# junfeng-chen/position_induced_transformer

Hardware: AMD Instinct MI355X
Metric: PiT fwd+bwd samples/sec on Darcy2D (higher is better)
Workload: dtype f32; 1 GPU; darcy2d 43x43 grid->16x16 latent, pit_fixed hid64 H2 blocks4 loc0.02, RelL2 (train_darcy.py:64-111), fwd+loss+bwd, per-GPU batch 8; per_gpu_batch=8, global_batch=8, parallelism=single, launch=hipgraph, head_scale_route=host

## Files before the change

### include/pit_hip.h

```cpp
#ifndef PIT_HIP_H
#define PIT_HIP_H

#ifdef __cplusplus
extern "C" {
#endif

#define PIT_ABI_VERSION 31
#define PIT_MAX_SPACE_DIM 8
#define PIT_DSCALE_SLOTS 1024

#define PIT_METRIC_EUCLID     0
#define PIT_METRIC_PERIODIC1D 1
#define PIT_METRIC_PERIODIC2D 2

#define PIT_ERR_NULL     -1
#define PIT_ERR_SIZE     -2
#define PIT_ERR_METRIC   -3
#define PIT_ERR_UNSUPPORTED -4

int pit_version(void);
const char* pit_error_string(int code);

#define PIT_MATH_FP32 0
#define PIT_MATH_BF16 1
// ... 339 lines not shown
                                   float* d_values, long ld_dvalues, long dvalues_bstride,
                                   const int* nbr_cnt, int nbr_cap, int coord_dims, void* stream);

int pit_distmat_select_fwd(const float* m, long ld_m, long m_bstride, int mesh_batch, int n_out, int n_in,
                           int rank_k, int need_kth, float* stats, void* stream);
int pit_distmat_fwd(const float* m, long ld_m, long m_bstride, int n_out, int n_in,
                    const float* values, int batch, int dim, long ld_values, long values_bstride,
                    const float* head, int n_head, int head_is_scale,
                    const float* stats, float rank_w, int masked,
                    float* out, long ld_out, long out_bstride, int out_col0, int copy_inputs,
                    float* rowstat, float* scale_out, int math_mode, void* stream);
long pit_distmat_bwd_workspace(int batch, int n_out, int n_head);
int pit_distmat_bwd(const float* m, long ld_m, long m_bstride, int n_out, int n_in,
                    const float* values, int batch, int dim, long ld_values, long values_bstride,
                    const float* head, int n_head, int head_is_scale, const float* scale,
                    const float* rowstat, int masked,
                    const float* d_out, long ld_dout, long dout_bstride, int out_col0,
                    float* d_values, long ld_dvalues, long dvalues_bstride, int add_residual,
                    float* d_head, int accumulate_head, double* workspace,
                    float* d_m, const float* out, long ld_out, long out_bstride, float* a_workspace,
                    int math_mode, void* stream);

#define PIT_HAS_DISTLIST 1
#define PIT_DISTLIST_MAX_CAP 2048
#define PIT_DISTLIST_CHUNK 512
#define PIT_DISTLIST_CHUNK_SLOTS(n_out, cap) ((long)(n_out) * (long)(cap) / (PIT_DISTLIST_CHUNK / 2) + 1)
int pit_distlist_select_fwd(const int* idx, const float* sqd, long ld, long bstride, int cap, int mesh_batch, int n_out, int n_in,
                            int rank_k, int need_kth, float* stats, void* stream);
int pit_distlist_fwd(const int* idx, const float* sqd, long ld, long bstride, int cap, int n_out, int n_in,
                     const float* values, int batch, int dim, long ld_values, long values_bstride,
                     const float* head, int n_head, int head_is_scale,
                     const float* stats, float rank_w, int masked,
                     float* out, long ld_out, long out_bstride, int out_col0, int copy_inputs,
                     float* rowstat, float* scale_out, int math_mode, void* stream);
long pit_distlist_bwd_workspace(int batch, int n_out, int cap, int dim);
int pit_distlist_bwd(const int* idx, const float* sqd, long ld, long bstride, int cap, int n_out, int n_in,
                     const float* values, int batch, int dim, long ld_values, long values_bstride,
                     const float* head, int n_head, int head_is_scale, const float* scale,
                     const float* rowstat, int masked,
                     const float* d_out, long ld_dout, long dout_bstride, int out_col0,
                     float* d_values, long ld_dvalues, long dvalues_bstride, int add_residual,
                     float* d_head, int accumulate_head, double* workspace,
                     float* d_sqd, const float* out, long ld_out, long out_bstride,
                     const int* rev_ptr, const int* rev_pos, const int* chunk_ptr, const int* chunk_key, float* dv_workspace,
                     int math_mode, void* stream);

#define PIT_HAS_RAGGED_STEP 1
int pit_rel_lp_loss_ragged_fwd_grad(const float* tru, const float* pred, const int* len, int batch, int npts, int nch, int p,
                                    float* norms, float* loss, unsigned* workspace, float* d_pred_unit, float* clear_buf,
                                    long clear_n, void* stream);
int pit_rel_max_norm_ragged(const float* tru, const float* pred, const int* len, int batch, int npts, int nch, float* out,
                            void* stream);

int pit_debug_mfma_tile(const float* a, const float* b, float* d, void* stream);

#define PIT_RIDER_OWN          0
#define PIT_RIDER_PAIR_DW      1
#define PIT_RIDER_PAIR_WIDE    2
#define PIT_RIDER_SPARSE_PAIR  3
#define PIT_RIDER_SPARSE_ROWS  4
#define PIT_RIDER_DHEAD_FINISH 5
#define PIT_RIDER_BLOCK        6
#define PIT_RIDER_BLOCK2       7
#define PIT_RIDER_SATT         8
#define PIT_RIDER_KINDS        9
int pit_debug_rider_counts(int* out, int n, int reset);

#define PIT_GEMM_RD_TN1            0
#define PIT_GEMM_RD_TN2            1
#define PIT_GEMM_RD_PAIR           2
#define PIT_GEMM_RD_TRIPLE_TN1     3
#define PIT_GEMM_RD_TRIPLE_TN2     4
#define PIT_GEMM_LDS_32            5
#define PIT_GEMM_LDS_64            6
#define PIT_GEMM_LDS_128           7
#define PIT_GEMM_LDS_AGZ           8
#define PIT_GEMM_BFL_32            9
#define PIT_GEMM_BFL_64           10
#define PIT_GEMM_BFL_128          11
#define PIT_GEMM_BFL_IO16         12
#define PIT_GEMM_RR               13
#define PIT_GEMM_RR_PAIR          14
#define PIT_GEMM_MUL_GELU_GRAD    15
#define PIT_GEMM_THIN_DZ1         16
#define PIT_GEMM_THIN_FWD         17
#define PIT_GEMM_THIN_FWD_STREAM  18
#define PIT_GEMM_THIN_DW          19
#define PIT_GEMM_MLP_FWD16        20
#define PIT_GEMM_MLP_BWD16        21
#define PIT_GEMM_MLP_FWD64        22
#define PIT_GEMM_MLP_FWD64_THIN   23
#define PIT_GEMM_MLP_BWD64        24
#define PIT_GEMM_MLP_BWD64_THIN   25
#define PIT_GEMM_LAST_FWD16       26
#define PIT_GEMM_LAST_BWD16       27
#define PIT_GEMM_LAST_FWD64       28
#define PIT_GEMM_LAST_BWD64       29
#define PIT_GEMM_KINDS            30
int pit_debug_gemm_counts(int* out, int n, int reset);

#ifdef __cplusplus
}
#endif
#endif
```

### position_induced_transformer_amd/_lib.py

```python
from __future__ import annotations

import ctypes
import os

import torch

_HERE = os.path.dirname(os.path.abspath(__file__))
LIB_PATH = os.environ.get("PIT_LIB_PATH") or os.path.join(_HERE, "csrc", "libpit_hip.so")

_P = ctypes.c_void_p
_I = ctypes.c_int
_L = ctypes.c_long
_F = ctypes.c_float

class MlpParamsJob(ctypes.Structure):
    _fields_ = [("x", _P), ("ldx", _L), ("rows", _I), ("n0", _I), ("n1", _I), ("n2", _I), ("h", _P), ("out_gelu", _I),
                ("d_y", _P), ("ld_dy", _L), ("d_w1", _P), ("d_b1", _P), ("d_w2", _P), ("d_b2", _P),
                ("accumulate", _I), ("scratch", _P), ("math_mode", _I)]


class BlockWeightsJob(ctypes.Structure):
    _fields_ = [("mesh", _P), ("n_pts", _I), ("space_dim", _I), ("metric", _I), ("period", _F),
                ("n_layers", _I), ("heads", _P), ("head_is_scale", _I), ("n_head", _I),
                ("e", _P), ("q", _P), ("inv", _P), ("rowstat", _P), ("scale_out", _P)]
# ... 102 lines not shown
    "pit_union_att_supported": [_I, _I, _I, _I],
    "pit_union_att_fwd": [_P, _P, _L, _L, _I, _I, _I, _P, _P, _L, _L, _I, _I, _P],
    "pit_union_att_bwd": [_P, _P, _L, _L, _I, _I, _I, _P, _P, _P, _L, _L, _I, _P, _L, _L, _P, _I, _P],
    "pit_encoder_fwd": [_P, _P, _I, _I, _P, _L, _L, _I, _I, _I, _I, _P, _I, _P, _P, _P, _P,
                        _P, _P, _P, _P, _P, _L, _P, _P, _P, _L, _P, _P, _P],
    "pit_encoder_bwd": [_P, _P, _I, _I, _P, _L, _L, _I, _I, _I, _I, _P, _P, _P, _P, _P, _P, _P, _L, _P, _P, _P],
    "pit_posatt_pre_supported": [_I, _I, _I, _I],
    "pit_posatt_pre_fwd": [_P, _P, _I, _I, _I, _I, _P, _L, _L, _P, _L, _L, _I, _I, _I, _P],
    "pit_posatt_pre_bwd": [_P, _P, _P, _I, _I, _I, _I, _P, _L, _L, _P, _L, _L, _I, _P, _L, _L, _I, _P, _I, _P],
    "pit_block_bwd": [_P, _P, _P, _I, _I, _I, _I, _P, _P, _P, _P, _P, _P, _P, _I, _I, _P, _L, _P, _P, _L, _P, _P, _I, _P],
    "pit_mlp_bf16_io_supported": [_I, _I, _I, _I, _I],
    "pit_mlp_fwd": [_P, _L, _I, _I, _I, _I, _P, _P, _P, _P, _I, _P, _P, _P, _P, _L, _I, _P],
    "pit_mlp_bwd": [_P, _L, _I, _I, _I, _I, _P, _P, _P, _P, _P, _I, _P, _L,
                    _P, _L, _P, _P, _P, _P, _I, _P, _I, _P],
    "pit_mlp_bwd_data": [_I, _I, _I, _I, _P, _P, _P, _P, _I, _P, _L, _P, _L, _P, _I, _P],
    "pit_mlp_bwd_params": [_P, _L, _I, _I, _I, _I, _P, _I, _P, _L, _P, _P, _P, _P, _I, _P, _I, _P],
    "pit_mlp_bwd_params_ordered": [_P, _L, _I, _I, _I, _I, _P, _I, _P, _L, _P, _P, _P, _P, _I, _P, _P, _P],
    "pit_mlp_bwd_params_ordered_workspace": [_I, _I, _I, _I],
    "pit_mlp_bwd_params_ordered_mfma": [_P, _L, _I, _I, _I, _I, _P, _I, _P, _L, _P, _P, _P, _P, _I, _P, _P, _P],
    "pit_mlp_bwd_params_ordered_mfma_workspace": [_I, _I, _I, _I],
    "pit_lists_sort_ranges": [_P, _P, _I, _I, _L, _P, _P],
    "pit_posatt_overflow_dv_ordered": [_P, _P, _I, _I, _I, _I, _I, _F, _I, _I, _P, _I, _I, _P, _P,
                                       _P, _L, _L, _I, _P, _L, _L, _P, _I, _I, _P],
    "pit_mlp_bwd_params_deferrable": [_I, _I, _I, _I, _I, _L],
    "pit_rel_lp_loss_fwd": [_P, _P, _P, _P, _I, _I, _I, _I, _P, _P, _P, _P],
    "pit_rel_lp_loss_fwd_grad": [_P, _P, _P, _P, _I, _I, _I, _I, _P, _P, _P, _P, _P, _P, _L, _P],
    "pit_rel_lp_loss_fwd_grad_ordered": [_P, _P, _P, _P, _I, _I, _I, _I, _P, _P, _P, _P, _P, _P, _L, _P],
    "pit_rel_lp_loss_bwd": [_P, _P, _P, _P, _I, _I, _I, _I, _P, _P, _P, _P, _P],
    "pit_plan_ragged_fwd": [_P, _P, _I, _I, _I, _I, _P, _P, _F, _I, _P, _P, _I, _P, _P, _P],
    "pit_posatt_ragged_fwd": _RAGGED + _FWD_RAGGED,
    "pit_posatt_ragged_bwd": _RAGGED + _BWD_RAGGED,
    "pit_plan_ragged_strided_fwd": [_P, _P, _I, _I, _I, _I, _L, _L, _P, _P, _F, _I, _P, _P, _I, _P, _P, _P],
    "pit_posatt_ragged_strided_fwd": _RAGGED_STRIDED + _FWD_RAGGED,
    "pit_posatt_ragged_strided_bwd": _RAGGED_STRIDED + _BWD_RAGGED,
    "pit_rel_lp_loss_ragged_fwd": [_P, _P, _P, _I, _I, _I, _I, _P, _P, _P],
    "pit_rel_lp_loss_ragged_bwd": [_P, _P, _P, _I, _I, _I, _I, _P, _P, _P, _P],
    "pit_rel_lp_loss_ragged_fwd_grad": [_P, _P, _P, _I, _I, _I, _I, _P, _P, _P, _P, _P, _L, _P],
    "pit_rel_max_norm_ragged": [_P, _P, _P, _I, _I, _I, _P, _P],
    "pit_distmat_select_fwd": [_P, _L, _L, _I, _I, _I, _I, _I, _P, _P],
    "pit_distmat_fwd": _MAT + _FWD_DIST,
    "pit_distmat_bwd_workspace": [_I, _I, _I],
    "pit_distmat_bwd": _MAT + _BWD_DIST + [_P] + _SAVED_OUT + [_P] + _TAIL,
    "pit_distlist_select_fwd": [_P, _P, _L, _L, _I, _I, _I, _I, _I, _I, _P, _P],
    "pit_distlist_fwd": _LIST + _FWD_DIST,
    "pit_distlist_bwd_workspace": [_I, _I, _I, _I],
    "pit_distlist_bwd": _LIST + _BWD_DIST + [_P] + _SAVED_OUT + [_P] * 5 + _TAIL,
    "pit_rel_max_norm": [_P, _P, _I, _I, _I, _P, _P, _P],
    "pit_instance_norm_fwd": [_P, _L, _L, _I, _I, _I, _F, _P, _P, _P],
    "pit_instance_norm_bwd": [_P, _P, _P, _I, _I, _I, _P, _P],
    "pit_adam_step": [_P, _P, _P, _P, _L, _P, _F, _F, _I, _F, _F, _F, _F, _I, _P, _P],
    "pit_debug_mfma_tile": [_P, _P, _P, _P],
    "pit_debug_rider_counts": [_P, _I, _I],
    "pit_debug_gemm_counts": [_P, _I, _I],
}

LONG_RETURN = {"pit_satt_tiles_elems", "pit_posatt_dmesh_workspace", "pit_mlp_bwd_params_ordered_workspace",
               "pit_mlp_bwd_params_ordered_mfma_workspace", "pit_distmat_bwd_workspace", "pit_distlist_bwd_workspace"}
ADDED_LATER = {"pit_distlist_select_fwd", "pit_distlist_fwd", "pit_distlist_bwd_workspace", "pit_distlist_bwd",
               "pit_rel_lp_loss_ragged_fwd_grad", "pit_rel_max_norm_ragged"}
DISTLIST_CHUNK = 512


def distlist_chunk_slots(n_out: int, cap: int) -> int:
    return int(n_out) * int(cap) // (DISTLIST_CHUNK // 2) + 1
ABI_VERSION = 31

_lib = None


def lib() -> ctypes.CDLL:
    global _lib
    if _lib is None:
        if not os.path.exists(LIB_PATH):
            raise RuntimeError(
                f"{LIB_PATH} not found: build it with `python -m position_induced_transformer_amd.build` "
                "(hipcc --offload-arch=gfx950). There is no CPU or PyTorch fallback for the PiT hot path.")
        handle = ctypes.CDLL(LIB_PATH)
        for name, argtypes in SIGNATURES.items():
            try:
                fn = getattr(handle, name)
            except AttributeError:
                if name not in ADDED_LATER:
                    raise
                raise RuntimeError(f"{LIB_PATH} was built before {name} joined PIT_ABI_VERSION {ABI_VERSION}: "
                                   "rebuild it (python -m position_induced_transformer_amd.build)") from None
            fn.argtypes = argtypes
            fn.restype = ctypes.c_char_p if name == "pit_error_string" else (_L if name in LONG_RETURN else _I)
        got = handle.pit_version()
        if got != ABI_VERSION:
            raise RuntimeError(f"{LIB_PATH} implements PIT_ABI_VERSION {got}, this package binds version {ABI_VERSION}: "
                               "rebuild it (python -m position_induced_transformer_amd.build)")
        _lib = handle
    return _lib


def check(code: int, what: str) -> None:
    if code != 0:
        msg = lib().pit_error_string(code)
        raise RuntimeError(f"{what} failed ({code}): {msg.decode() if msg else '?'}")


def stream_ptr() -> int:
    return torch.cuda.current_stream().cuda_stream


def ptr(t) -> int:
    return 0 if t is None else t.data_ptr()


def values_args(t, with_batch: bool) -> tuple:
    b, _, d = t.shape
    return (t.data_ptr(),) + ((b, d) if with_batch else (d,)) + (t.stride(1), t.stride(0))
# ... 25 lines not shown
```

### position_induced_transformer_amd/csrc/pit_block.hip

```cpp
#include "pit_common.h"
#include "pit_gemm_rd.h"
#include "pit_block_dev.h"
#include <cstdlib>

namespace {

#ifdef PIT_STAMPS
__device__ unsigned long long pit_block_stamps[32];
#define BSTAMP(i_) do { if (blockIdx.x == 5 && threadIdx.x == 0) pit_block_stamps[i_] = __builtin_amdgcn_s_memtime(); } while (0)
#else
#define BSTAMP(i_) do { } while (0)
#endif

#ifdef PIT_WGREC
__device__ unsigned long long pit_block_wgrec[1024 * 4];
#define BREC(slot_) do { if (threadIdx.x == 0 && blockIdx.x < 1024) {                                                       \
        pit_block_wgrec[blockIdx.x * 4 + (slot_)] = __builtin_amdgcn_s_memrealtime();                                       \
        if ((slot_) == 0) { pit_block_wgrec[blockIdx.x * 4 + 2] = __builtin_amdgcn_s_getreg((4 << 0) | (0 << 6) | (31 << 11));   \
                            pit_block_wgrec[blockIdx.x * 4 + 3] = __builtin_amdgcn_s_getreg((20 << 0) | (0 << 6) | (31 << 11)); } } } while (0)
#else
#define BREC(slot_) do { } while (0)
#endif
#ifdef PIT_STAMPS_DBG
__device__ int pit_block_dbg = 0;
#define PIT_BLOCK_DBG pit_block_dbg
#else
#define PIT_BLOCK_DBG 0
#endif
#ifndef PIT_BLOCK_EXP
#define PIT_BLOCK_EXP 0
#endif

__global__ __launch_bounds__(256) void block_weights_kernel(WeightsArgs a) { block_weights_body(a, blockIdx.x); }

template <int NH, bool SHARED>
__device__ __forceinline__ void slab_contract(const float* __restrict__ w, long wstride, int L, const float* __restrict__ v,
                                              long ldv, int vhead, const float* __restrict__ sc, int jb, int je, int l15, int kq,
                                              f32x4_t (&acc)[SHARED ? NH : 1][4]) {
    constexpr int NS = SHARED ? 2 : 1;
    const float* wp = w + (long)l15 * L + 4 * kq;
    const float* vp = v + 4 * l15;
    for (int j0 = jb; j0 < je; j0 += 16 * NS) {
        float4 av[NH][NS], sv[NH][NS], bv[SHARED ? 1 : NH][NS][4];
        const int dbg = PIT_BLOCK_DBG;
#pragma unroll
        for (int h = 0; h < NH; ++h)
#pragma unroll
            for (int s = 0; s < NS; ++s) {
                av[h][s] = (dbg & 4) ? make_float4(1.f, 2.f, 3.f, 4.f) : *reinterpret_cast<const float4*>(wp + h * wstride + j0 + 16 * s);
                if (!SHARED) sv[h][s] = *reinterpret_cast<const float4*>(sc + (long)h * L + j0 + 16 * s + 4 * kq);
            }
#pragma unroll
        for (int h = 0; h < (SHARED ? 1 : NH); ++h)
#pragma unroll
            for (int s = 0; s < NS; ++s)
#pragma unroll
                for (int m = 0; m < 4; ++m)
                    bv[h][s][m] = (dbg & 2) ? make_float4(1.f, 2.f, 3.f, 4.f)
                                            : *reinterpret_cast<const float4*>(vp + h * vhead + (long)(j0 + 16 * s + 4 * kq + m) * ldv);
        __builtin_amdgcn_sched_barrier(0);
#pragma unroll
        for (int s = 0; s < NS; ++s)
#pragma unroll
            for (int m = 0; m < 4; ++m)
#pragma unroll
                for (int h = 0; h < NH; ++h) {
                    if ((PIT_BLOCK_EXP & (SHARED ? 1 : 4)) && (SHARED ? s == 1 : h == 1)) {
                        asm volatile("" :: "v"(av[h][s].x), "v"(av[h][s].y), "v"(av[h][s].z), "v"(av[h][s].w));
                        asm volatile("" :: "v"(bv[SHARED ? 0 : h][s][m].x), "v"(bv[SHARED ? 0 : h][s][m].y), "v"(bv[SHARED ? 0 : h][s][m].z), "v"(bv[SHARED ? 0 : h][s][m].w));
                        if (!SHARED) asm volatile("" :: "v"(sv[h][s].x), "v"(sv[h][s].y), "v"(sv[h][s].z), "v"(sv[h][s].w));
                        continue;
                    }
                    const float* ap = &av[h][s].x;
                    const float* sp = &sv[h][s].x;
                    const float aw = SHARED ? ap[m] : ap[m] * sp[m];
                    const float4 bb = bv[SHARED ? 0 : h][s][m];
                    f32x4_t (&ac)[4] = acc[SHARED ? h : 0];
                    ac[0] = mfma_16x16x4(aw, bb.x, ac[0]);
                    ac[1] = mfma_16x16x4(aw, bb.y, ac[1]);
                    ac[2] = mfma_16x16x4(aw, bb.z, ac[2]);
                    ac[3] = mfma_16x16x4(aw, bb.w, ac[3]);
                }
    }
}

__device__ __forceinline__ bool slab_of(int id, int batch, int slabs, int& sample, int& slab) {
    if (PIT_BLOCK_DBG & 1) return slab_of_linear(id, batch, slabs, sample, slab);
    return slab_of_xcd(id, batch, slabs, sample, slab);
}

struct BlockFwdArgs {
    const float *e, *inv;
    int L, batch;
    float* xcat;
    const float *w1, *b1, *w2, *b2;
    int out_gelu;
    float *z1, *h, *z2, *y; long ldy;
};

template <int H, bool WLDS>
__global__ __launch_bounds__(512, WLDS ? 1 : 2) void block_fwd_kernel(BlockFwdArgs g) {
    constexpr int W = (1 + H) * BD;
    constexpr int XP = W + 4, HP = BD + 4;
    constexpr int KS = W / 16;
    constexpr int NW1 = BD * W / 4 / 512, NW2 = BD * BD / 4 / 512;
    extern __shared__ __attribute__((aligned(16))) float smem[];
    float* pk = smem;
    float* xs = smem + H * PARK_FLOATS;
    float* hs = xs + 16 * XP;
    float* w1s = hs + 16 * HP;
    float* w2s = w1s + BD * XP;
    const int tid = threadIdx.x, lane = tid & 63, wave = tid >> 6;
    const int l15 = lane & 15, kq = lane >> 4;
    const int slabs = g.L / 16;
    int b, slab;
    if (!slab_of(blockIdx.x, g.batch, slabs, b, slab)) return;
    const int n0 = slab * 16;
    const long m0 = ((long)b * slabs + slab) * 16;
    const int klen = g.L / BW;

    float4 xown = make_float4(0.f, 0.f, 0.f, 0.f);
    if (tid < 256) xown = *reinterpret_cast<const float4*>(g.xcat + (m0 + (tid >> 4)) * W + 4 * (tid & 15));
    const float rinv0 = g.inv[(long)((tid >> 8) % H) * g.L + n0 + 4 * ((tid & 63) >> 4) + ((tid >> 6) & 3)];

    BSTAMP(0);
    const bool mlp_wave = wave < 4;
    const int c1 = (wave & 3) * 16 + l15;
    float4 bv[KS], w2v[4];
    float bias = 0.0f, bias2 = 0.0f;
    auto load_weights = [&]() {
        if (!mlp_wave) return;
        if (!WLDS) {
#pragma unroll
            for (int s = 0; s < KS; ++s) bv[s] = *reinterpret_cast<const float4*>(g.w1 + (long)c1 * W + 16 * s + 4 * kq);
#pragma unroll
            for (int s = 0; s < 4; ++s) w2v[s] = *reinterpret_cast<const float4*>(g.w2 + (long)c1 * BD + 16 * s + 4 * kq);
        }
        bias = g.b1[c1];
        bias2 = g.b2[c1];
    };
    f32x4_t wq1[WLDS ? NW1 : 1], wq2[WLDS ? NW2 : 1];
    if (WLDS) {
#pragma unroll
        for (int p = 0; p < NW1; ++p) wq1[p] = reinterpret_cast<const f32x4_t*>(g.w1)[p * 512 + tid];
#pragma unroll
        for (int p = 0; p < NW2; ++p) wq2[p] = reinterpret_cast<const f32x4_t*>(g.w2)[p * 512 + tid];
        load_weights();
    }
    f32x4_t acc[H][4];
#pragma unroll
    for (int hh = 0; hh < H; ++hh)
#pragma unroll
        for (int t = 0; t < 4; ++t) acc[hh][t] = f32x4_t{0.f, 0.f, 0.f, 0.f};
    constexpr int EP = 256 + 4;
    const bool elds = WLDS && g.L == 256 && !(PIT_BLOCK_EXP & 64);
    if (elds) {
        float* es = w1s;
        const float* vp = g.xcat + (long)b * g.L * W + 4 * l15;
        const int j0 = wave * 32;
        f32x4_t eq[H * 2];
#pragma unroll
        for (int p = 0; p < H * 2; ++p) {
            const int q = p * 512 + tid;
            eq[p] = *reinterpret_cast<const f32x4_t*>(g.e + (long)(q >> 10) * g.L * g.L + (long)(n0 + ((q >> 6) & 15)) * g.L + 4 * (q & 63));
        }
        f32x4_t bvv[2][4];
#pragma unroll
        for (int s = 0; s < 2; ++s)
#pragma unroll
            for (int m = 0; m < 4; ++m) bvv[s][m] = *reinterpret_cast<const f32x4_t*>(vp + (long)(j0 + 16 * s + 4 * kq + m) * W);
        __builtin_amdgcn_sched_barrier(0);
#pragma unroll
        for (int p = 0; p < H * 2; ++p) {
            const int q = p * 512 + tid;
            *reinterpret_cast<f32x4_t*>(es + ((q >> 10) * 16 + ((q >> 6) & 15)) * EP + 4 * (q & 63)) = eq[p];
        }
        __syncthreads();
#pragma unroll
        for (int s = 0; s < 2; ++s) {
            f32x4_t av[H];
#pragma unroll
            for (int hh = 0; hh < H; ++hh) av[hh] = *reinterpret_cast<const f32x4_t*>(es + (hh * 16 + l15) * EP + j0 + 16 * s + 4 * kq);
#pragma unroll
            for (int m = 0; m < 4; ++m)
#pragma unroll
                for (int hh = 0; hh < H; ++hh) {
                    acc[hh][0] = mfma_16x16x4(av[hh][m], bvv[s][m][0], acc[hh][0]);
                    acc[hh][1] = mfma_16x16x4(av[hh][m], bvv[s][m][1], acc[hh][1]);
                    acc[hh][2] = mfma_16x16x4(av[hh][m], bvv[s][m][2], acc[hh][2]);
                    acc[hh][3] = mfma_16x16x4(av[hh][m], bvv[s][m][3], acc[hh][3]);
                }
        }
    } else {
        slab_contract<H, true>(g.e + (long)n0 * g.L, (long)g.L * g.L, g.L, g.xcat + (long)b * g.L * W, W, 0, nullptr,
                               wave * klen, (wave + 1) * klen, l15, kq, acc);
    }
    BSTAMP(1);
    if (!WLDS) load_weights();
#pragma unroll
    for (int hh = 0; hh < H; ++hh) park(pk, wave * H + hh, lane, acc[hh]);
    if (tid < 256) *reinterpret_cast<float4*>(xs + (tid >> 4) * XP + 4 * (tid & 15)) = xown;
    __syncthreads();
    BSTAMP(2);
    for (int item = tid; item < H * 256; item += 512) {
        const int hh = item >> 8, i = (item >> 6) & 3, ln = item & 63;
        const int r = 4 * (ln >> 4) + i, col = 4 * (ln & 15);
        float4 s = parked_sum(pk, hh, BW, H, i, ln);
        const float rinv = item == tid ? rinv0 : g.inv[(long)hh * g.L + n0 + r];
        s.x *= rinv; s.y *= rinv; s.z *= rinv; s.w *= rinv;
        *reinterpret_cast<float4*>(xs + r * XP + BD + hh * BD + col) = s;
        *reinterpret_cast<float4*>(g.xcat + (m0 + r) * W + BD + hh * BD + col) = s;
    }
    if (WLDS) {
#pragma unroll
        for (int p = 0; p < NW1; ++p) {
            const int q = p * 512 + tid, row = q / (W / 4), c4 = q % (W / 4);
            *reinterpret_cast<f32x4_t*>(w1s + row * XP + 4 * c4) = wq1[p];
        }
#pragma unroll
        for (int p = 0; p < NW2; ++p) {
            const int q = p * 512 + tid, row = q / (BD / 4), c4 = q % (BD / 4);
            *reinterpret_cast<f32x4_t*>(w2s + row * HP + 4 * c4) = wq2[p];
        }
    }
    BSTAMP(3);
    __syncthreads();
    BSTAMP(4);
    if (mlp_wave) {
        f32x4_t a0 = {0.f, 0.f, 0.f, 0.f}, a1 = {0.f, 0.f, 0.f, 0.f};
#pragma unroll
        for (int s = 0; s < KS; ++s) {
            if ((PIT_BLOCK_EXP & 2) && (s & 1)) { if (!WLDS) asm volatile("" :: "v"(bv[s].x), "v"(bv[s].y), "v"(bv[s].z), "v"(bv[s].w)); continue; }
            const float4 a = *reinterpret_cast<const float4*>(xs + l15 * XP + 16 * s + 4 * kq);
            const float4 bw = WLDS ? *reinterpret_cast<const float4*>(w1s + c1 * XP + 16 * s + 4 * kq) : bv[s];
            a0 = mfma_16x16x4(a.x, bw.x, a0);
            a1 = mfma_16x16x4(a.y, bw.y, a1);
            a0 = mfma_16x16x4(a.z, bw.z, a0);
            a1 = mfma_16x16x4(a.w, bw.w, a1);
        }
        BSTAMP(5);
#pragma unroll
        for (int i = 0; i < 4; ++i) {
            const int r = 4 * kq + i;
            const float z = a0[i] + a1[i] + bias;
            const float hv = gelu_erf(z);
            hs[r * HP + c1] = hv;
            g.z1[(m0 + r) * BD + c1] = z;
            g.h[(m0 + r) * BD + c1] = hv;
        }
    }
    BSTAMP(6);
    __syncthreads();
    BSTAMP(7);
    if (!mlp_wave) return;
    f32x4_t o0 = {0.f, 0.f, 0.f, 0.f}, o1 = {0.f, 0.f, 0.f, 0.f};
#pragma unroll
    for (int s = 0; s < 4; ++s) {
        const float4 a = *reinterpret_cast<const float4*>(hs + l15 * HP + 16 * s + 4 * kq);
        const float4 bw = WLDS ? *reinterpret_cast<const float4*>(w2s + c1 * HP + 16 * s + 4 * kq) : w2v[s];
        o0 = mfma_16x16x4(a.x, bw.x, o0);
        o1 = mfma_16x16x4(a.y, bw.y, o1);
        o0 = mfma_16x16x4(a.z, bw.z, o0);
        o1 = mfma_16x16x4(a.w, bw.w, o1);
    }
    BSTAMP(8);
#pragma unroll
    for (int i = 0; i < 4; ++i) {
        const long r = m0 + 4 * kq + i;
        float v = o0[i] + o1[i] + bias2;
        if (g.out_gelu) { g.z2[r * BD + c1] = v; v = gelu_erf(v); }
        g.y[r * g.ldy + c1] = v;
    }
    BSTAMP(9);
}

struct BlockBwdArgs {
    const float *e, *inv, *qw;
    int L, batch;
    const float* d_xcat;
    const float* xcat;
    double* dscale;
    const float *w1, *w2, *z1, *z2; int out_gelu, n0p;
    float *d_xprev; long ld_dxprev;
    float *dz1, *dz2;
    float* d_values; long ld_dvalues;
    int n_chain, n_ds;
};

template <int H>
__device__ __forceinline__ void block_bwd_chain(const BlockBwdArgs& g, float* smem, int slab) {
    constexpr int W = (1 + H) * BD;
    constexpr int P1 = BD + 4;
    float* pk = smem;
    float* ds2 = smem + PARK_FLOATS;
    float* ds1 = ds2 + 16 * P1;
    const int tid = threadIdx.x, lane = tid & 63, wave = tid >> 6;
    const int l15 = lane & 15, kq = lane >> 4;
    const int slabs = g.L / 16;
    int b, sl;
    if (!slab_of(slab, g.batch, slabs, b, sl)) return;
    const int j0 = sl * 16;
    const long m0 = ((long)b * slabs + sl) * 16;
    const int klen = g.L / BW;

    const int oi = (tid >> 6) & 3, oln = tid & 63, oh = tid >> 8;
    const int orow = 4 * (oln >> 4) + oi, ocol = 4 * (oln & 15) + 2 * oh;
    const bool has_mlp = g.w1 != nullptr;
    const float2 res = *reinterpret_cast<const float2*>(g.d_xcat + (m0 + orow) * W + ocol);
    float2 z2v = make_float2(0.f, 0.f);
    if (has_mlp && g.out_gelu) z2v = *reinterpret_cast<const float2*>(g.z2 + (m0 + orow) * BD + ocol);
    const int c1 = (wave & 3) * 16 + l15;
    BSTAMP(10);
    f32x4_t acc[1][4];
#pragma unroll
    for (int t = 0; t < 4; ++t) acc[0][t] = f32x4_t{0.f, 0.f, 0.f, 0.f};
    slab_contract<H, false>(g.e + (long)j0 * g.L, (long)g.L * g.L, g.L, g.d_xcat + (long)b * g.L * W + BD, W, BD, g.inv,
                            wave * klen, (wave + 1) * klen, l15, kq, acc);
    BSTAMP(11);
    float w2v[4][4], z1v[4], w1v[2][4][4];
    if (has_mlp) {
// ... 94 lines not shown
    const int tid = threadIdx.x, lane = tid & 63, wave = tid >> 6;
    const int l15 = lane & 15, kq = lane >> 4;
    const int slabs = g.L / 16;
    int b, sl;
    if (!slab_of(slab, g.batch, slabs, b, sl)) return;
    const int n0 = sl * 16;
    const long m0 = ((long)b * slabs + sl) * 16;
    const int klen = g.L / BW;
    const bool own = tid < H * 256;
    const int hh = tid >> 8, i = (tid >> 6) & 3, ln = tid & 63;
    const int r = 4 * (ln >> 4) + i, col = 4 * (ln & 15);
    float4 dov = make_float4(0.f, 0.f, 0.f, 0.f);
    if (own) dov = *reinterpret_cast<const float4*>(g.d_xcat + (m0 + r) * W + BD + hh * BD + col);
    f32x4_t acc[H][4];
#pragma unroll
    for (int h2 = 0; h2 < H; ++h2)
#pragma unroll
        for (int t = 0; t < 4; ++t) acc[h2][t] = f32x4_t{0.f, 0.f, 0.f, 0.f};
    slab_contract<H, true>(g.qw + (long)n0 * g.L, (long)g.L * g.L, g.L, g.xcat + (long)b * g.L * W, W, 0, nullptr,
                           wave * klen, (wave + 1) * klen, l15, kq, acc);
#pragma unroll
    for (int h2 = 0; h2 < H; ++h2) park(pk, wave * H + h2, lane, acc[h2]);
    __syncthreads();
    double part = 0.0;
    if (own) {
        const float4 s = parked_sum(pk, hh, BW, H, i, ln);
        part = (double)s.x * (double)dov.x + (double)s.y * (double)dov.y + (double)s.z * (double)dov.z + (double)s.w * (double)dov.w;
    }
    part = wave_sum_d(part);
    if (lane == 0) wred[wave] = part;
    __syncthreads();
    if (tid < H) {
        double tot = 0.0;
        for (int w = 4 * tid; w < 4 * tid + 4; ++w) tot += wred[w];
        atomicAdd(g.dscale + (long)tid * PIT_DSCALE_SLOTS + ((int)(m0 >> 4) & (PIT_DSCALE_SLOTS - 1)), -tot);
    }
}

template <int H, int NDW>
__global__ __launch_bounds__(512) void block_bwd_kernel(BlockBwdArgs g, pit_detail::DwPair w, pit_detail::DwPair w2) {
    extern __shared__ __attribute__((aligned(16))) float smem[];
    int id = blockIdx.x;
    BREC(0);
    if (id < g.n_chain) { block_bwd_chain<H>(g, smem, id); BREC(1); return; }
    id -= g.n_chain;
    if (id < g.n_ds) { block_bwd_dscale<H>(g, smem, id); BREC(1); return; }
    id -= g.n_ds;
    if (PIT_BLOCK_EXP & 32) return;
    if (NDW >= 1 && id < w.n1 + w.n2) { dw_pair_body(w, id, smem); BREC(1); return; }
    if (NDW >= 2) dw_pair_body(w2, id - (w.n1 + w.n2), smem);
    BREC(1);
}

constexpr size_t fwd_smem(int H, bool wlds) {
    return ((size_t)H * PARK_FLOATS + 16 * ((1 + H) * BD + 4) + 16 * (BD + 4) + (wlds ? BD * ((1 + H) * BD + 4) + BD * (BD + 4) : 0)) * sizeof(float);
}
constexpr size_t bwd_smem(int H, bool dscale) {
    return std::max((size_t)(PARK_FLOATS + 2 * 16 * (BD + 4)) * sizeof(float),
                    dscale ? ((size_t)H * PARK_FLOATS) * sizeof(float) + BW * sizeof(double) : (size_t)0);
}

}

extern "C" int pit_block_supported(int n_pts, int n_head, int dim, int batch) {
    if (dim != BD || (n_head != 1 && n_head != 2)) return 0;
    if (n_pts <= 0 || batch <= 0 || n_pts % (32 * BW) != 0) return 0;
    if (n_pts > 2048) return 0;
    const long rows = (long)batch * n_pts;
    return rows >= 256 && rows <= 16384;
}

extern "C" int pit_block_weights(const float* mesh, int n_pts, int space_dim, int metric, float period, int n_layers,
                                 const float* const* heads, int head_is_scale, int n_head, float* e, float* q,
                                 float* inv, float* rowstat, float* scale_out, void* stream) {
    WeightsArgs a;
    if (int rc = fill_weights_args(a, mesh, n_pts, space_dim, metric, period, n_layers, heads, head_is_scale, n_head, e, q, inv,
                                   rowstat, scale_out)) return rc;
    const long rows = (long)n_layers * n_head * n_pts;
    hipLaunchKernelGGL(block_weights_kernel, dim3((unsigned)((rows + 3) / 4)), dim3(256), 0, (hipStream_t)stream, a);
    PIT_CHECK_LAUNCH();
    return 0;
}

extern "C" int pit_block_fwd(const float* e, const float* inv, int n_pts, int n_head, int dim, int batch, float* xcat,
                             const float* w1, const float* b1, const float* w2, const float* b2, int out_gelu,
                             float* z1, float* h, float* z2, float* y, long ldy, int math_mode, void* stream) {
    if (!e || !inv || !xcat || !w1 || !b1 || !w2 || !b2 || !z1 || !h || !y || (out_gelu && !z2)) return PIT_ERR_NULL;
    if (math_mode != PIT_MATH_FP32 || !pit_block_supported(n_pts, n_head, dim, batch)) return PIT_ERR_UNSUPPORTED;
    if (ldy < dim || !aligned16(e) || !aligned16(xcat) || !aligned16(w1) || !aligned16(w2)) return PIT_ERR_SIZE;
    BlockFwdArgs g;
    g.e = e; g.inv = inv; g.L = n_pts; g.batch = batch; g.xcat = xcat;
    g.w1 = w1; g.b1 = b1; g.w2 = w2; g.b2 = b2; g.out_gelu = out_gelu;
    g.z1 = z1; g.h = h; g.z2 = z2; g.y = y; g.ldy = ldy;
    const dim3 grid((unsigned)slab_grid(batch, n_pts / 16)), block(64 * BW);
    static const bool no_wlds = getenv("PIT_NO_BLOCK_WLDS") != nullptr;
    static const int n_cus = [] {
        int dev = 0, cus = 0;
        if (hipGetDevice(&dev) != hipSuccess || hipDeviceGetAttribute(&cus, hipDeviceAttributeMultiprocessorCount, dev) != hipSuccess) cus = 0;
        return cus;
    }();
    const bool earlyw = !no_wlds && (int)grid.x <= n_cus;
    const size_t FWD_SMEM = fwd_smem(n_head, earlyw);
#define PIT_BLOCK_FWD(H_, E_)                                                                                              \
    do {                                                                                                                   \
        static bool once = ((void)hipFuncSetAttribute((const void*)block_fwd_kernel<H_, E_>,                              \
                                                hipFuncAttributeMaxDynamicSharedMemorySize, 160 * 1024), true);            \
        (void)once;                                                                                                        \
        hipLaunchKernelGGL((block_fwd_kernel<H_, E_>), grid, block, FWD_SMEM, (hipStream_t)stream, g);                     \
    } while (0)
    if (n_head == 1) { if (earlyw) PIT_BLOCK_FWD(1, true); else PIT_BLOCK_FWD(1, false); }
    else { if (earlyw) PIT_BLOCK_FWD(2, true); else PIT_BLOCK_FWD(2, false); }
#undef PIT_BLOCK_FWD
    PIT_CHECK_LAUNCH();
    return 0;
}

#ifdef PIT_WGREC
extern "C" int pit_block_read_wgrec(unsigned long long* out, int n) {
    return (int)hipMemcpyFromSymbol(out, HIP_SYMBOL(pit_block_wgrec), (size_t)n * 4 * sizeof(unsigned long long));
}
#endif
#ifdef PIT_STAMPS_DBG
extern "C" int pit_block_set_dbg(int v) { return (int)hipMemcpyToSymbol(HIP_SYMBOL(pit_block_dbg), &v, sizeof(int)); }
#endif
#ifdef PIT_STAMPS
extern "C" int pit_block_read_stamps(unsigned long long* out) {
    return (int)hipMemcpyFromSymbol(out, HIP_SYMBOL(pit_block_stamps), sizeof(unsigned long long) * 32);
}
#endif

extern "C" int pit_block_bwd(const float* e, const float* inv, const float* qw, int n_pts, int n_head, int dim, int batch,
                             const float* d_xcat, const float* xcat, double* dscale,
                             const float* w1, const float* w2, const float* z1, const float* z2, int out_gelu, int n0_prev,
                             float* d_xprev, long ld_dxprev, float* scratch_prev,
                             float* d_values, long ld_dvalues,
                             const pit_mlp_params_job* rider, const pit_mlp_params_job* rider2, int math_mode, void* stream) {
    if (!e || !inv || !d_xcat) return PIT_ERR_NULL;
    if (dscale && (!qw || !xcat)) return PIT_ERR_NULL;
    if (math_mode != PIT_MATH_FP32 || !pit_block_supported(n_pts, n_head, dim, batch)) return PIT_ERR_UNSUPPORTED;
    const bool has_mlp = w1 != nullptr;
    if (has_mlp) {
        if (!w2 || !z1 || !scratch_prev || (out_gelu && !z2)) return PIT_ERR_NULL;
        if (n0_prev <= 0 || n0_prev > 16 * 16 || (d_xprev && ld_dxprev < n0_prev)) return PIT_ERR_SIZE;
    } else if (!d_values || ld_dvalues < dim || ld_dvalues % 4 != 0 || !aligned16(d_values)) {
        return d_values ? PIT_ERR_SIZE : PIT_ERR_NULL;
    }
    if (!aligned16(e) || !aligned16(d_xcat) || (qw && !aligned16(qw)) || (xcat && !aligned16(xcat)) ||
        (has_mlp && (!aligned16(scratch_prev) || (z2 && !aligned16(z2))))) return PIT_ERR_SIZE;
    hipStream_t s = (hipStream_t)stream;
    const long rows = (long)batch * n_pts;
    BlockBwdArgs g;
    g.e = e; g.inv = inv; g.qw = qw; g.L = n_pts; g.batch = batch; g.d_xcat = d_xcat; g.xcat = xcat; g.dscale = dscale;
    g.w1 = w1; g.w2 = w2; g.z1 = z1; g.z2 = z2; g.out_gelu = out_gelu; g.n0p = n0_prev;
    g.d_xprev = d_xprev; g.ld_dxprev = ld_dxprev;
    g.dz1 = scratch_prev; g.dz2 = has_mlp ? scratch_prev + rows * dim : nullptr;
    g.d_values = d_values; g.ld_dvalues = ld_dvalues;
    g.n_chain = slab_grid(batch, n_pts / 16);
    g.n_ds = dscale ? g.n_chain : 0;
    pit_detail::DwPair dw = pit_detail::DwPair(), dw2 = pit_detail::DwPair();
    const pit_mlp_params_job* jobs[2] = {rider, rider2};
    pit_detail::DwPair* plans[2] = {&dw, &dw2};
    int ndw = 0;
    bool carried[2] = {false, false};
    for (int r = 0; r < 2; ++r)
        if (jobs[r] && pit_detail::plan_dw_pair(*jobs[r], BW, plans[ndw], 768, true)) { carried[r] = true; ++ndw; }
    const int n_dw = (ndw >= 1 ? dw.n1 + dw.n2 : 0) + (ndw >= 2 ? dw2.n1 + dw2.n2 : 0);
    const bool any_rr = (ndw >= 1 && (dw.rr1 || dw.rr2)) || (ndw >= 2 && (dw2.rr1 || dw2.rr2));
    const size_t sm = std::max(std::max(bwd_smem(n_head, dscale != nullptr), ndw ? (size_t)BW * 16 * 64 * sizeof(float) : (size_t)0),
// ... 26 lines not shown
```

Baseline: 55930 samples/s.

## Add 8-row stacked-head slab form for two-head block forward kernel

Adds a block forward variant that processes 8 rows per workgroup with both heads stacked into a single 16-row MFMA tile. This doubles the number of workgroups so more CUs are used when the grid is small (batch 8, 256 latent points). E is always staged through LDS, and the MLP stage runs on a half-empty padded tile. The variant is selected by default when the doubled grid still fits within the CU count. Each workgroup reloads the weights, so weight-load traffic doubles and half the MLP MFMA work is wasted.

```diff
diff --git a/include/pit_hip.h b/include/pit_hip.h
--- a/include/pit_hip.h
+++ b/include/pit_hip.h
@@ -415,6 +415,10 @@
 int pit_rel_max_norm_ragged(const float* tru, const float* pred, const int* len, int batch, int npts, int nch, float* out,
                             void* stream);
 
+#define PIT_HAS_BLOCK_ROWS8 1
+int pit_block_fwd_set_form(int form);
+int pit_block_fwd_last_rows(void);
+
 int pit_debug_mfma_tile(const float* a, const float* b, float* d, void* stream);
 
 #define PIT_RIDER_OWN          0
diff --git a/position_induced_transformer_amd/_lib.py b/position_induced_transformer_amd/_lib.py
--- a/position_induced_transformer_amd/_lib.py
+++ b/position_induced_transformer_amd/_lib.py
@@ -178,12 +178,15 @@
     "pit_debug_mfma_tile": [_P, _P, _P, _P],
     "pit_debug_rider_counts": [_P, _I, _I],
     "pit_debug_gemm_counts": [_P, _I, _I],
+    "pit_block_fwd_set_form": [_I],
+    "pit_block_fwd_last_rows": [],
 }
 
 LONG_RETURN = {"pit_satt_tiles_elems", "pit_posatt_dmesh_workspace", "pit_mlp_bwd_params_ordered_workspace",
                "pit_mlp_bwd_params_ordered_mfma_workspace", "pit_distmat_bwd_workspace", "pit_distlist_bwd_workspace"}
 ADDED_LATER = {"pit_distlist_select_fwd", "pit_distlist_fwd", "pit_distlist_bwd_workspace", "pit_distlist_bwd",
-               "pit_rel_lp_loss_ragged_fwd_grad", "pit_rel_max_norm_ragged"}
+               "pit_rel_lp_loss_ragged_fwd_grad", "pit_rel_max_norm_ragged",
+               "pit_block_fwd_set_form", "pit_block_fwd_last_rows"}
 DISTLIST_CHUNK = 512
 
 
diff --git a/position_induced_transformer_amd/csrc/pit_block.hip b/position_induced_transformer_amd/csrc/pit_block.hip
--- a/position_induced_transformer_amd/csrc/pit_block.hip
+++ b/position_induced_transformer_amd/csrc/pit_block.hip
@@ -1,6 +1,7 @@
 #include "pit_common.h"
 #include "pit_gemm_rd.h"
 #include "pit_block_dev.h"
+#include <atomic>
 #include <cstdlib>
 
 namespace {
@@ -98,30 +99,34 @@
     float *z1, *h, *z2, *y; long ldy;
 };
 
-template <int H, bool WLDS>
+template <int H, bool WLDS, bool R8 = false>
 __global__ __launch_bounds__(512, WLDS ? 1 : 2) void block_fwd_kernel(BlockFwdArgs g) {
+    static_assert(!R8 || (H == 2 && WLDS), "the stacked form: two heads, weights and E through LDS");
     constexpr int W = (1 + H) * BD;
     constexpr int XP = W + 4, HP = BD + 4;
     constexpr int KS = W / 16;
     constexpr int NW1 = BD * W / 4 / 512, NW2 = BD * BD / 4 / 512;
+    constexpr int RS = R8 ? 8 : 16;
+    constexpr int NA = R8 ? 1 : H;
     extern __shared__ __attribute__((aligned(16))) float smem[];
     float* pk = smem;
-    float* xs = smem + H * PARK_FLOATS;
+    float* xs = smem + NA * PARK_FLOATS;
     float* hs = xs + 16 * XP;
     float* w1s = hs + 16 * HP;
     float* w2s = w1s + BD * XP;
     const int tid = threadIdx.x, lane = tid & 63, wave = tid >> 6;
     const int l15 = lane & 15, kq = lane >> 4;
-    const int slabs = g.L / 16;
+    const int slabs = g.L / RS;
     int b, slab;
     if (!slab_of(blockIdx.x, g.batch, slabs, b, slab)) return;
-    const int n0 = slab * 16;
-    const long m0 = ((long)b * slabs + slab) * 16;
+    const int n0 = slab * RS;
+    const long m0 = ((long)b * slabs + slab) * RS;
     const int klen = g.L / BW;
 
     float4 xown = make_float4(0.f, 0.f, 0.f, 0.f);
-    if (tid < 256) xown = *reinterpret_cast<const float4*>(g.xcat + (m0 + (tid >> 4)) * W + 4 * (tid & 15));
-    const float rinv0 = g.inv[(long)((tid >> 8) % H) * g.L + n0 + 4 * ((tid & 63) >> 4) + ((tid >> 6) & 3)];
+    if (tid < RS * 16) xown = *reinterpret_cast<const float4*>(g.xcat + (m0 + (tid >> 4)) * W + 4 * (tid & 15));
+    const int r0 = 4 * ((tid & 63) >> 4) + ((tid >> 6) & 3);
+    const float rinv0 = R8 ? g.inv[(long)(r0 >> 3) * g.L + n0 + (r0 & 7)] : g.inv[(long)((tid >> 8) % H) * g.L + n0 + r0];
 
     BSTAMP(0);
     const bool mlp_wave = wave < 4;
@@ -147,22 +152,23 @@
         for (int p = 0; p < NW2; ++p) wq2[p] = reinterpret_cast<const f32x4_t*>(g.w2)[p * 512 + tid];
         load_weights();
     }
-    f32x4_t acc[H][4];
-#pragma unroll
-    for (int hh = 0; hh < H; ++hh)
+    f32x4_t acc[NA][4];
+#pragma unroll
+    for (int hh = 0; hh < NA; ++hh)
 #pragma unroll
         for (int t = 0; t < 4; ++t) acc[hh][t] = f32x4_t{0.f, 0.f, 0.f, 0.f};
     constexpr int EP = 256 + 4;
-    const bool elds = WLDS && g.L == 256 && !(PIT_BLOCK_EXP & 64);
+    const bool elds = R8 || (WLDS && g.L == 256 && !(PIT_BLOCK_EXP & 64));
     if (elds) {
         float* es = w1s;
         const float* vp = g.xcat + (long)b * g.L * W + 4 * l15;
         const int j0 = wave * 32;
-        f32x4_t eq[H * 2];
-#pragma unroll
-        for (int p = 0; p < H * 2; ++p) {
+        constexpr int NE = H * RS / 8;
+        f32x4_t eq[NE];
+#pragma unroll
+        for (int p = 0; p < NE; ++p) {
             const int q = p * 512 + tid;
-            eq[p] = *reinterpret_cast<const f32x4_t*>(g.e + (long)(q >> 10) * g.L * g.L + (long)(n0 + ((q >> 6) & 15)) * g.L + 4 * (q & 63));
+            eq[p] = *reinterpret_cast<const f32x4_t*>(g.e + (long)(q / (64 * RS)) * g.L * g.L + (long)(n0 + ((q >> 6) & (RS - 1))) * g.L + 4 * (q & 63));
         }
         f32x4_t bvv[2][4];
 #pragma unroll
@@ -171,43 +177,53 @@
             for (int m = 0; m < 4; ++m) bvv[s][m] = *reinterpret_cast<const f32x4_t*>(vp + (long)(j0 + 16 * s + 4 * kq + m) * W);
         __builtin_amdgcn_sched_barrier(0);
 #pragma unroll
-        for (int p = 0; p < H * 2; ++p) {
+        for (int p = 0; p < NE; ++p) {
             const int q = p * 512 + tid;
-            *reinterpret_cast<f32x4_t*>(es + ((q >> 10) * 16 + ((q >> 6) & 15)) * EP + 4 * (q & 63)) = eq[p];
+            *reinterpret_cast<f32x4_t*>(es + (q >> 6) * EP + 4 * (q & 63)) = eq[p];
         }
         __syncthreads();
 #pragma unroll
         for (int s = 0; s < 2; ++s) {
-            f32x4_t av[H];
-#pragma unroll
-            for (int hh = 0; hh < H; ++hh) av[hh] = *reinterpret_cast<const f32x4_t*>(es + (hh * 16 + l15) * EP + j0 + 16 * s + 4 * kq);
+            f32x4_t av[NA];
+#pragma unroll
+            for (int hh = 0; hh < NA; ++hh) av[hh] = *reinterpret_cast<const f32x4_t*>(es + (hh * 16 + l15) * EP + j0 + 16 * s + 4 * kq);
 #pragma unroll
             for (int m = 0; m < 4; ++m)
 #pragma unroll
-                for (int hh = 0; hh < H; ++hh) {
+                for (int hh = 0; hh < NA; ++hh) {
                     acc[hh][0] = mfma_16x16x4(av[hh][m], bvv[s][m][0], acc[hh][0]);
                     acc[hh][1] = mfma_16x16x4(av[hh][m], bvv[s][m][1], acc[hh][1]);
                     acc[hh][2] = mfma_16x16x4(av[hh][m], bvv[s][m][2], acc[hh][2]);
                     acc[hh][3] = mfma_16x16x4(av[hh][m], bvv[s][m][3], acc[hh][3]);
                 }
         }
-    } else {
+    } else if constexpr (!R8) {
         slab_contract<H, true>(g.e + (long)n0 * g.L, (long)g.L * g.L, g.L, g.xcat + (long)b * g.L * W, W, 0, nullptr,
                                wave * klen, (wave + 1) * klen, l15, kq, acc);
     }
     BSTAMP(1);
     if (!WLDS) load_weights();
 #pragma unroll
-    for (int hh = 0; hh < H; ++hh) park(pk, wave * H + hh, lane, acc[hh]);
-    if (tid < 256) *reinterpret_cast<float4*>(xs + (tid >> 4) * XP + 4 * (tid & 15)) = xown;
+    for (int hh = 0; hh < NA; ++hh) park(pk, wave * NA + hh, lane, acc[hh]);
+    if (tid < RS * 16) *reinterpret_cast<float4*>(xs + (tid >> 4) * XP + 4 * (tid & 15)) = xown;
+    if (R8)
+        for (int q = tid; q < 8 * XP / 4; q += 512) reinterpret_cast<float4*>(xs + 8 * XP)[q] = make_float4(0.f, 0.f, 0.f, 0.f);
     __syncthreads();
     BSTAMP(2);
-    for (int item = tid; item < H * 256; item += 512) {
-        const int hh = item >> 8, i = (item >> 6) & 3, ln = item & 63;
-        const int r = 4 * (ln >> 4) + i, col = 4 * (ln & 15);
-        float4 s = parked_sum(pk, hh, BW, H, i, ln);
-        const float rinv = item == tid ? rinv0 : g.inv[(long)hh * g.L + n0 + r];
-        s.x *= rinv; s.y *= rinv; s.z *= rinv; s.w *= rinv;
+    if (!R8) {
+        for (int item = tid; item < H * 256; item += 512) {
+            const int hh = item >> 8, i = (item >> 6) & 3, ln = item & 63;
+            const int r = 4 * (ln >> 4) + i, col = 4 * (ln & 15);
+            float4 s = parked_sum(pk, hh, BW, H, i, ln);
+            const float rinv = item == tid ? rinv0 : g.inv[(long)hh * g.L + n0 + r];
+            s.x *= rinv; s.y *= rinv; s.z *= rinv; s.w *= rinv;
+            *reinterpret_cast<float4*>(xs + r * XP + BD + hh * BD + col) = s;
+            *reinterpret_cast<float4*>(g.xcat + (m0 + r) * W + BD + hh * BD + col) = s;
+        }
+    } else if (tid < 256) {
+        const int hh = r0 >> 3, r = r0 & 7, col = 4 * (tid & 15);
+        float4 s = parked_sum(pk, 0, BW, 1, (tid >> 6) & 3, tid & 63);
+        s.x *= rinv0; s.y *= rinv0; s.z *= rinv0; s.w *= rinv0;
         *reinterpret_cast<float4*>(xs + r * XP + BD + hh * BD + col) = s;
         *reinterpret_cast<float4*>(g.xcat + (m0 + r) * W + BD + hh * BD + col) = s;
     }
@@ -245,8 +261,10 @@
             const float z = a0[i] + a1[i] + bias;
             const float hv = gelu_erf(z);
             hs[r * HP + c1] = hv;
-            g.z1[(m0 + r) * BD + c1] = z;
-            g.h[(m0 + r) * BD + c1] = hv;
+            if (!R8 || kq < 2) {
+                g.z1[(m0 + r) * BD + c1] = z;
+                g.h[(m0 + r) * BD + c1] = hv;
+            }
         }
     }
     BSTAMP(6);
@@ -266,6 +284,7 @@
     BSTAMP(8);
 #pragma unroll
     for (int i = 0; i < 4; ++i) {
+        if (R8 && kq >= 2) break;
         const long r = m0 + 4 * kq + i;
         float v = o0[i] + o1[i] + bias2;
         if (g.out_gelu) { g.z2[r * BD + c1] = v; v = gelu_erf(v); }
@@ -466,13 +485,16 @@
     BREC(1);
 }
 
-constexpr size_t fwd_smem(int H, bool wlds) {
-    return ((size_t)H * PARK_FLOATS + 16 * ((1 + H) * BD + 4) + 16 * (BD + 4) + (wlds ? BD * ((1 + H) * BD + 4) + BD * (BD + 4) : 0)) * sizeof(float);
+constexpr size_t fwd_smem(int H, bool wlds, bool r8) {
+    return ((size_t)(r8 ? 1 : H) * PARK_FLOATS + 16 * ((1 + H) * BD + 4) + 16 * (BD + 4) + (wlds ? BD * ((1 + H) * BD + 4) + BD * (BD + 4) : 0)) * sizeof(float);
 }
 constexpr size_t bwd_smem(int H, bool dscale) {
     return std::max((size_t)(PARK_FLOATS + 2 * 16 * (BD + 4)) * sizeof(float),
                     dscale ? ((size_t)H * PARK_FLOATS) * sizeof(float) + BW * sizeof(double) : (size_t)0);
 }
+
+std::atomic<int> block_fwd_form{0};
+std::atomic<int> block_fwd_rows{0};
 
 }
 
@@ -506,28 +528,41 @@
     g.e = e; g.inv = inv; g.L = n_pts; g.batch = batch; g.xcat = xcat;
     g.w1 = w1; g.b1 = b1; g.w2 = w2; g.b2 = b2; g.out_gelu = out_gelu;
     g.z1 = z1; g.h = h; g.z2 = z2; g.y = y; g.ldy = ldy;
-    const dim3 grid((unsigned)slab_grid(batch, n_pts / 16)), block(64 * BW);
     static const bool no_wlds = getenv("PIT_NO_BLOCK_WLDS") != nullptr;
+    static const bool no_rows8 = [] { const char* v = getenv("PIT_BLOCK_ROWS8"); return v && v[0] == '0'; }();
     static const int n_cus = [] {
         int dev = 0, cus = 0;
         if (hipGetDevice(&dev) != hipSuccess || hipDeviceGetAttribute(&cus, hipDeviceAttributeMultiprocessorCount, dev) != hipSuccess) cus = 0;
         return cus;
     }();
-    const bool earlyw = !no_wlds && (int)grid.x <= n_cus;
-    const size_t FWD_SMEM = fwd_smem(n_head, earlyw);
-#define PIT_BLOCK_FWD(H_, E_)                                                                                              \
+    const int form = block_fwd_form.load(std::memory_order_relaxed);
+    const bool rows8 = n_head == 2 && n_pts == 256 && !no_wlds && form != 16 && (form == 8 || !no_rows8) &&
+                       slab_grid(batch, n_pts / 8) <= n_cus;
+    const dim3 grid((unsigned)slab_grid(batch, n_pts / (rows8 ? 8 : 16))), block(64 * BW);
+    const bool earlyw = rows8 || (!no_wlds && (int)grid.x <= n_cus);
+    const size_t FWD_SMEM = fwd_smem(n_head, earlyw, rows8);
+#define PIT_BLOCK_FWD(...)                                                                                                 \
     do {                                                                                                                   \
-        static bool once = ((void)hipFuncSetAttribute((const void*)block_fwd_kernel<H_, E_>,                              \
+        static bool once = ((void)hipFuncSetAttribute((const void*)block_fwd_kernel<__VA_ARGS__>,                         \
                                                 hipFuncAttributeMaxDynamicSharedMemorySize, 160 * 1024), true);            \
         (void)once;                                                                                                        \
-        hipLaunchKernelGGL((block_fwd_kernel<H_, E_>), grid, block, FWD_SMEM, (hipStream_t)stream, g);                     \
+        hipLaunchKernelGGL((block_fwd_kernel<__VA_ARGS__>), grid, block, FWD_SMEM, (hipStream_t)stream, g);                \
     } while (0)
     if (n_head == 1) { if (earlyw) PIT_BLOCK_FWD(1, true); else PIT_BLOCK_FWD(1, false); }
+    else if (rows8) PIT_BLOCK_FWD(2, true, true);
     else { if (earlyw) PIT_BLOCK_FWD(2, true); else PIT_BLOCK_FWD(2, false); }
 #undef PIT_BLOCK_FWD
     PIT_CHECK_LAUNCH();
+    block_fwd_rows.store(rows8 ? 8 : 16, std::memory_order_relaxed);
     return 0;
 }
+
+extern "C" int pit_block_fwd_set_form(int form) {
+    if (form != 0 && form != 8 && form != 16) return PIT_ERR_SIZE;
+    return block_fwd_form.exchange(form, std::memory_order_relaxed);
+}
+
+extern "C" int pit_block_fwd_last_rows(void) { return block_fwd_rows.load(std::memory_order_relaxed); }
 
 #ifdef PIT_WGREC
 extern "C" int pit_block_read_wgrec(unsigned long long* out, int n) {
```

Result: faster. 57650 samples/s, median of 6 (+3.1%).
